# barrust/pyprobables

Measured on AMD Instinct MI355X. Metric: million keys/sec insert+lookup (Bloom m=2^28 k=7, CMS 2^20x5), higher is better.
Workload: dtype u64; 1 GPU; cfg2 Bloom m=2^28 k=7: per rank per step clear + insert 10M 16B keys + (merge) + check them; keys_per_rank=10000000, key_bytes=16, m_bits=268435456, k=7, parallelism=single GPU

## Files before the change

pyprobables_amd/csrc/psk_capi.hip:

```cpp
#include "psk_host.hpp"

#include <map>
#include <mutex>
#include <utility>

static thread_local char g_err[512] = "";

int fail(int code, const char *fmt, ...)
{
    va_list ap;
    va_start(ap, fmt);
    vsnprintf(g_err, sizeof(g_err), fmt, ap);
    va_end(ap);
    return code;
}


extern "C" const char *psk_last_error(void) { return g_err; }
extern "C" int psk_version(void) { return 100; }

extern "C" int psk_device_count(int *count)
{
    if (!count) return fail(PSK_EINVAL, "count is NULL");
    int n = 0;
// ... 317 lines not shown
    if (logical_bytes) *logical_bytes = s->logical_bytes;
    return PSK_OK;
}

extern "C" int psk_read_table(psk_sketch *s, void *dst_host, uint64_t nbytes, void *stream)
{
    CHECK_HANDLE_RO(s, -1);
    if (!dst_host || nbytes > s->padded_bytes) return fail(PSK_EINVAL, "bad read_table arguments");
    hipStream_t st = (hipStream_t)stream;
    PSK_TRY(flush_combined(s, st));
    HIP_TRY(hipMemcpyAsync(dst_host, s->table, nbytes, hipMemcpyDeviceToHost, st));
    HIP_TRY(hipStreamSynchronize(st));
    return PSK_OK;
}

extern "C" int psk_write_table(psk_sketch *s, const void *src_host, uint64_t nbytes, void *stream)
{
    CHECK_HANDLE(s, -1);
    if (!src_host || nbytes > s->padded_bytes) return fail(PSK_EINVAL, "bad write_table arguments");
    hipStream_t st = (hipStream_t)stream;
    PSK_TRY(drop_pending(s, st));
    s->clear_pending = false;
    HIP_TRY(hipMemsetAsync(s->table, 0, s->padded_bytes, st));
    HIP_TRY(hipMemcpyAsync(s->table, src_host, nbytes, hipMemcpyHostToDevice, st));
    HIP_TRY(hipMemsetAsync(s->ctr, 0, sizeof(long long) * PSK_CTR_COUNT, st));
    if (s->kind != PSK_KIND_BLOOM) {
        const uint64_t nel = s->logical_bytes / 4;
        hipLaunchKernelGGL(k_absmax, dim3(grid_for_keys(nel)), dim3(kBlock), 0, st, (const uint32_t *)s->table, nel,
                           s->kind == PSK_KIND_CMS ? 1 : 0, s->ctr);
        HIP_TRY(hipGetLastError());
    }
    HIP_TRY(hipStreamSynchronize(st));
    return PSK_OK;
}

extern "C" int psk_rescan_bound(psk_sketch *s, void *stream)
{
    CHECK_HANDLE(s, -1);
    if (s->owns_table || s->table_private) s->shadow.exposed = false;
    if (s->kind == PSK_KIND_BLOOM) return PSK_OK;
    hipStream_t st = (hipStream_t)stream;
    PSK_TRY(flush_combined(s, st));
    HIP_TRY(hipMemsetAsync(s->ctr + PSK_CTR_ABS_BOUND, 0, sizeof(long long), st));
    const uint64_t nel = s->logical_bytes / 4;
    hipLaunchKernelGGL(k_absmax, dim3(grid_for_keys(nel)), dim3(kBlock), 0, st, (const uint32_t *)s->table, nel,
                       s->kind == PSK_KIND_CMS ? 1 : 0, s->ctr);
    HIP_TRY(hipGetLastError());
    return PSK_OK;
}

extern "C" int psk_get_counters(psk_sketch *s, int64_t out[PSK_CTR_COUNT], void *stream)
{
    CHECK_HANDLE_RO(s, -1);
    if (!out) return fail(PSK_EINVAL, "out is NULL");
    hipStream_t st = (hipStream_t)stream;
    PSK_TRY(flush_combined(s, st));
    HIP_TRY(hipMemcpyAsync(out, s->ctr, sizeof(long long) * PSK_CTR_COUNT, hipMemcpyDeviceToHost, st));
    HIP_TRY(hipStreamSynchronize(st));
    return PSK_OK;
}

extern "C" int psk_reset_counters(psk_sketch *s, void *stream)
{
    CHECK_HANDLE(s, -1);
    HIP_TRY(hipMemsetAsync(s->ctr, 0, sizeof(long long) * PSK_CTR_ABS_BOUND, (hipStream_t)stream));
    return PSK_OK;
}

int raise_dyn_lds(const void *kernel, size_t bytes)
{
    static std::mutex mu;
    static std::map<std::pair<const void *, int>, size_t> granted;
    int dev = 0;
    HIP_TRY(hipGetDevice(&dev));
    std::lock_guard<std::mutex> lock(mu);
    size_t &have = granted[{kernel, dev}];
    if (bytes > have) {
        HIP_TRY(hipFuncSetAttribute(kernel, hipFuncAttributeMaxDynamicSharedMemorySize, (int)bytes));
        have = bytes;
    }
    return PSK_OK;
}

extern "C" int psk_set_option(const char *name, int64_t value)
{
    if (!name) return fail(PSK_EINVAL, "option name is NULL");
    const OptDesc *d = opt_find(name);
    if (!d || d->cls == kOptReadOnly) return fail(PSK_EINVAL, d ? "option %s is read-only" : "unknown option %s", name);
    if (value < d->lo) value = d->lo;
    __atomic_store_n(d->var, value, __ATOMIC_RELAXED);
    return PSK_OK;
}

extern "C" int psk_debug_phase_profile(psk_sketch *s, uint32_t nbuckets, uint32_t nwg, uint64_t out[12])
{
    if (!s || !s->s_cnt.p) return fail(PSK_EINVAL, "no partition scratch yet");
    PSK_USE_DEVICE(s->device);
    HIP_TRY(hipDeviceSynchronize());
    char *p = (char *)s->s_cnt.p + (size_t)nbuckets * nwg * 4;
    HIP_TRY(hipMemcpy(out, p, 96, hipMemcpyDeviceToHost));
    HIP_TRY(hipMemset(p, 0, 96));
    return PSK_OK;
}

extern "C" int psk_sketch_set_option(psk_sketch *s, const char *name, int64_t value)
{
    if (!s || !name) return fail(PSK_EINVAL, "NULL argument");
    if (!strcmp(name, "table_private")) {
        s->table_private = value != 0;
        if (s->table_private) s->shadow.exposed = false;
        else if (!s->owns_table) s->shadow.exposed = true;
        if (s->shadow.exposed && s->clear_pending) {
            PSK_USE_DEVICE(s->device);
            PSK_TRY(clear_materialize(s, nullptr));
        }
        ++s->table_version;
        return PSK_OK;
    }
    const OptDesc *d = opt_find(name);
    if (!d || d->ho < 0) return fail(PSK_EINVAL, "%s is not a per-sketch option", name);
    if (value != kHoUnset && value < d->lo) value = d->lo;
    s->opt[d->ho] = value;
    return PSK_OK;
}

extern "C" int psk_sketch_get_option(psk_sketch *s, const char *name, int64_t *value)
{
    if (!s || !name || !value) return fail(PSK_EINVAL, "NULL argument");
    if (!strcmp(name, "table_private")) {
        *value = s->table_private ? 1 : 0;
        return PSK_OK;
    }
    if (!strcmp(name, "window_pending_batches")) {
        *value = s->win.n ? (int64_t)s->win.batches.size() : 0;
        return PSK_OK;
    }
    const OptDesc *d = opt_find(name);
    if (!d || d->ho < 0) return fail(PSK_EINVAL, "%s is not a per-sketch option", name);
    *value = s->opt[d->ho] != kHoUnset ? s->opt[d->ho] : __atomic_load_n(d->var, __ATOMIC_RELAXED);
    return PSK_OK;
}

extern "C" int psk_get_option(const char *name, int64_t *value)
{
    if (!name || !value) return fail(PSK_EINVAL, "NULL argument");
    const OptDesc *d = opt_find(name);
    if (!d) return fail(PSK_EINVAL, "unknown option %s", name);
    *value = __atomic_load_n(d->var, __ATOMIC_RELAXED);
    return PSK_OK;
}

extern "C" int psk_scratch_bytes(psk_sketch *s, uint64_t bytes[3])
{
    if (!s || !bytes) return fail(PSK_EINVAL, "psk_scratch_bytes: NULL argument");
    uint64_t all = 0, waiting = 0;
    (void)for_each_scratch(s, [&](DevBuf &b, bool is_waiting) {
        if (b.p) all += b.cap;
        if (b.p && is_waiting) waiting += b.cap;
        return (int)PSK_OK;
    });
    bytes[0] = all;
    bytes[1] = waiting;
    bytes[2] = s->shadow.img.p ? s->shadow.img.cap : 0;
    return PSK_OK;
}

// ... 18 lines not shown
```

pyprobables_amd/csrc/psk_cbf.hip:

```cpp
#include "psk_stage.hpp"
#include "psk_nibble.hpp"
#include "psk_window.hpp"

static int cbf_apply_direct(psk_sketch *s, const Batch &b, const uint32_t *w, bool remove, hipStream_t st)
{
    unsigned long long *sat = (unsigned long long *)(s->ctr + PSK_CTR_SATURATED);
    return with_source(b, [&](auto src) {
        return with_pow2(s, [&](auto P) {
            if (remove) return launch_apply(src, CbfSub<P.value>{(uint32_t *)s->table, s->md, s->k, w, sat - 1}, b.n, st);
            return launch_apply(src, CbfAdd<P.value>{(uint32_t *)s->table, s->md, s->k, w, s->ctr, sat, false}, b.n, st);
        });
    });
}

static int cbf_apply_device(psk_sketch *s, const Batch &b, const uint32_t *w, bool remove, hipStream_t st)
{
    if (b.n == 0) return PSK_OK;
    PSK_TRY(post_acct(s, w, b.n, remove ? PSK_CTR_REMOVED : PSK_CTR_ADDED, (long long)s->k, st, !remove, false));
    bool done = false;
    PSK_TRY(remove ? cbf_remove_partitioned(s, b, w, st, &done, 0, nullptr) : cbf_add_partitioned(s, b, w, st, &done));
    PSK_TRY(settle_acct(s, w, b.n, st));
    if (done) return PSK_OK;
    return cbf_apply_direct(s, b, w, remove, st);
}

static int comb_order(psk_sketch *s, hipStream_t st)
{
    if (!s->scat.appended || st == s->scat.last) return PSK_OK;
    if (!s->scat.ev) HIP_TRY(hipEventCreateWithFlags(&s->scat.ev, hipEventDisableTiming));
    HIP_TRY(hipEventRecord(s->scat.ev, s->scat.last));
    HIP_TRY(hipStreamWaitEvent(st, s->scat.ev, 0));
    s->scat.last = st;
    return PSK_OK;
}

static int comb_appended(psk_sketch *s, hipStream_t st)
{
    s->scat.last = st;
    s->scat.appended = true;
    return PSK_OK;
}

static bool older_updates_pending(const psk_sketch *s)
{
    return s->comb.add.n || s->comb.rem.n || s->comb.badd.n() || s->comb.brem.n() || (s->scat.ready && s->scat.add.n);
}

static int scat_zero(psk_sketch *s, hipStream_t st)
{
    const uint64_t nseg = (uint64_t)s->scat.g.nbuckets * s->scat.g.nwg;
    if (!s->scat.add.cnt.p) return PSK_OK;
    hipLaunchKernelGGL(k_zero_u32, dim3(256), dim3(256), 0, st, (uint32_t *)s->scat.add.cnt.p, nseg);
    HIP_TRY(hipGetLastError());
    return PSK_OK;
}

static int scat_drop(psk_sketch *s, hipStream_t st)
{
    if (!s->scat.ready || s->scat.add.n == 0) return PSK_OK;
    PSK_TRY(comb_order(s, st));
    PSK_TRY(scat_zero(s, st));
    s->scat.add.n = 0;
    return PSK_OK;
}

int drop_pending(psk_sketch *s, hipStream_t st)
{
    s->comb.add.n = s->comb.rem.n = 0;
    s->comb.add.unit = s->comb.rem.unit = true;
    s->comb.badd.clear();
    s->comb.brem.clear();
    s->win.n = s->win.copied = 0;
    s->win.batches.clear();
    return scat_drop(s, st);
}

static int scat_flush(psk_sketch *s, hipStream_t st)
{
    if (!s->scat.ready || s->scat.add.n == 0) return PSK_OK;
    PSK_TRY(comb_order(s, st));
    const uint64_t na = s->scat.add.n;
    s->scat.add.n = 0;
    PartGeom g = s->scat.g;
    const uint64_t per_seg = (uint64_t)g.nbuckets * g.nwg * 6;
    g.dense = (na * s->k / per_seg) < (uint64_t)g_part_dense_groups ? 1u : 0u;
    const size_t lds = (size_t)1 << (g.shift - 1);
    unsigned long long *sat = (unsigned long long *)(s->ctr + PSK_CTR_SATURATED);
    const uint32_t direct = na * s->k >= s->m / 8 ? 0u : 1u;
    PSK_TRY(set_dyn_lds(k_nib_apply<0>, lds));
    hipLaunchKernelGGL(k_nib_apply<0>, dim3(g.nbuckets), dim3(kApplyThreads), lds, st, (uint32_t *)s->table, s->m, g, (const uint32_t *)s->scat.add.cnt.p,
                       (const uint4 *)s->scat.add.part.p, sat, direct);
    HIP_TRY(hipGetLastError());
    return scat_zero(s, st);
}

static int scat_append(psk_sketch *s, const Batch &b, uint64_t cap, hipStream_t st, bool *done)
{
    *done = false;
    {
        const uint64_t by_table = s->m * 5 / (2 * (uint64_t)(s->k ? s->k : 1));
        if (cap > by_table) cap = by_table;
    }
    if (s->kind != PSK_KIND_CBF || g_update_nibble == 0 || b.n == 0 || b.n > cap || s->k > 32) return PSK_OK;
    if (b.layout == PSK_KEYS_HASHES && b.key_len < s->k) return PSK_OK;
    if (!s->scat.ready || s->scat.cap != cap) {
        PartGeom g;
        if (!scat_geometry(s, cap, &g)) return PSK_OK;
        PSK_TRY(scat_flush(s, st));
        s->scat.g = g;
        s->scat.cap = cap;
        s->scat.ready = true;
    }
    psk_sketch::ScatList &l = s->scat.add;
    if (l.n + b.n > cap) PSK_TRY(flush_combined(s, st));
    const PartGeom &g = s->scat.g;
    const uint64_t part_bytes = (uint64_t)g.nbuckets * g.nwg * g.segcap * 16 + 256, cnt_bytes = (uint64_t)g.nbuckets * g.nwg * 4 + 128;
    if (l.part.cap < part_bytes || l.cnt.cap < cnt_bytes) {
        if (s->eff[HO_SCRATCH_BUDGET] > 0 && (int64_t)(part_bytes + cnt_bytes) > s->eff[HO_SCRATCH_BUDGET]) return PSK_OK;
        if (ensure(l.part, part_bytes) != PSK_OK || ensure(l.cnt, cnt_bytes) != PSK_OK) return PSK_OK;
        HIP_TRY(hipMemsetAsync(l.cnt.p, 0, cnt_bytes, st));
        l.n = 0;
    }
    PSK_TRY(comb_order(s, st));
    bool appended = false;
    PSK_TRY(cbf_scat_append(s, b, st, &appended));
    if (!appended) return PSK_OK;
    l.n += b.n;
    PSK_TRY(comb_appended(s, st));
    *done = true;
    return PSK_OK;
}

static int borrowed_flush(psk_sketch *s, psk_sketch::BorrowList &bl, bool remove, hipStream_t st)
{
    const uint64_t n = bl.n();
    if (n == 0) return PSK_OK;
    const uint32_t nb = (uint32_t)bl.base.size();
    PSK_TRY(ensure(s->s_brw, (uint64_t)(2 * nb + 2) * 8));
    const void **base_dev = (const void **)s->s_brw.p;
    uint64_t *start_dev = (uint64_t *)s->s_brw.p + nb;
    HIP_TRY(hipMemcpyAsync(base_dev, bl.base.data(), (size_t)nb * 8, hipMemcpyHostToDevice, st));
    HIP_TRY(hipMemcpyAsync(start_dev, bl.start.data(), (size_t)(nb + 1) * 8, hipMemcpyHostToDevice, st));
    HIP_TRY(hipStreamSynchronize(st));
    std::vector<const void *> bases;
    std::vector<uint64_t> starts;
    bases.swap(bl.base);
    starts.swap(bl.start);
    bl.clear();
    PSK_TRY(account_weights(s, (const uint32_t *)nullptr, n, remove ? PSK_CTR_REMOVED : PSK_CTR_ADDED, (long long)s->k, st, !remove));
    bool done = false;
    PSK_TRY(cbf_unit_multi_partitioned(s, (const void *const *)base_dev, start_dev, nb, n, remove ? 1 : 0, st, &done));
    if (done) return PSK_OK;
    for (uint32_t j = 0; j < nb; ++j) {
        const Batch b{PSK_KEYS_FIXED, bases[j], nullptr, starts[j + 1] - starts[j], 16};
        PSK_TRY(cbf_apply_direct(s, b, nullptr, remove, st));
    }
    return PSK_OK;
}

constexpr size_t kWinMaxBatches = 4096;

static uint64_t win_capacity(const psk_sketch *s)
{
    uint64_t cap = s->m / 2;
    if (cap < (1u << 20)) cap = 1u << 20;
    if (s->eff[HO_WINDOW_KEYS] > 0 && cap > (uint64_t)s->eff[HO_WINDOW_KEYS]) cap = (uint64_t)s->eff[HO_WINDOW_KEYS];
    cap = cap_round_by_budget(s, cap, 16.0 + (double)s->k * (16.0 / 6.0) * 1.5);
    return cap;
// ... 491 lines not shown
```

pyprobables_amd/csrc/psk_host.hpp:

```cpp
#pragma once
#include "psk_device.hpp"
#include "psk_partition.hpp"
#include "psk_part_bins.hpp"

#include <hip/hip_runtime.h>

#include <cstdarg>
#include <cstdio>
#include <cstdlib>
#include <cstring>
#include <new>
#include <type_traits>
#include <vector>

#include "../../include/psk.h"

using namespace psk;

#define PSK_HIDDEN __attribute__((visibility("hidden")))

PSK_HIDDEN int fail(int code, const char *fmt, ...);

#define HIP_TRY(expr)                                                                                   \
    do {                                                                                                \
// ... 158 lines not shown
        bool active = false, scattered = false;
        Batch b{};
        PartGeom g{};
        uint64_t round_keys = 0;
        int scheme = 0;
        uint32_t gen = 0;
    } pend;
};

PSK_HIDDEN int ensure(DevBuf &b, uint64_t bytes);

PSK_HIDDEN void resolve_options(psk_sketch *s);
#define CHECK_HANDLE_RO(s, want_kind)                                                    \
    do {                                                                                 \
        if (!(s)) return fail(PSK_EINVAL, "sketch handle is NULL");                      \
        if ((want_kind) >= 0 && (s)->kind != (want_kind))                                \
            return fail(PSK_EINVAL, "wrong sketch kind %d for this call", (s)->kind);    \
        resolve_options(s);                                                              \
    } while (0);                                                                         \
    PSK_USE_DEVICE((s)->device)
#define CHECK_HANDLE(s, want_kind)                                                       \
    CHECK_HANDLE_RO(s, want_kind);                                                       \
    ++(s)->table_version

static inline int grid_for_keys(uint64_t n)
{
    uint64_t g = (n + kBlock - 1) / kBlock;
    const uint64_t cap = 256ULL * 16;
    if (g > cap) g = cap;
    return (int)(g ? g : 1);
}


extern PSK_HIDDEN int64_t g_part_mode, g_part_max_keys, g_part_cache_bytes, g_part_two_level_slices, g_part_debug, g_part_tile_threads,
    g_part_even_tiles, g_part_dense_groups, g_part_bins, g_ragged_sort, g_lookup_half, g_lookup_nibble, g_update_nibble, g_nib_min_lg_lookup,
    g_nib_min_lg_update, g_small_weights, g_remove_dryrun, g_combine_keys, g_auto_combine_keys, g_window_wide, g_window_tile,
    g_window_force_fail, g_merge_single_rank, g_lazy_clear, g_host_poll_us,
    g_cbf_ordered_replays, g_window_folds, g_window_replays, g_small_weights_used, g_cbf_shadow_hits, g_running_fast, g_running_sequential,
    g_update_running_fast, g_update_running_sequential;

static inline bool part_slices(uint64_t cells, uint32_t max_shift, uint32_t min_shift, PartGeom *g,
                               uint64_t max_buckets = kPartMaxBuckets, int target_lg = 8)
{
    if (cells >= (1ULL << 32) || cells < (1ULL << 16)) return false;
    const uint32_t lg = 63 - __builtin_clzll(cells);
    int shift = (int)lg - target_lg;
    if (shift > (int)max_shift) shift = max_shift;
    if (shift < (int)min_shift) shift = min_shift;
    const uint64_t B = (cells + (1ULL << shift) - 1) >> shift;
    if (B > max_buckets) return false;
    g->nbuckets = (uint32_t)B;
    g->shift = (uint32_t)shift;
    g->dbg = (uint32_t)g_part_debug | (g_ragged_sort == 0 ? kGeomNoSortBit : 0u);
    g->split = g->split_idx = 0;
    g->dense = 0;
    g->append = 0;
    return true;
}

static inline bool nib_geometry(uint64_t cells, bool update, PartGeom *g)
{
    if (update ? cells <= (1ULL << g_nib_min_lg_update) : cells < (1ULL << g_nib_min_lg_lookup)) return false;
    return part_slices(cells, kNibShift, 15, g, kPartMaxBuckets, 8);
}

static inline bool nib_load_ok(uint64_t n, uint32_t k, uint64_t cells) { return n * (uint64_t)k * 2 <= cells * 5; }

static inline bool scat_geometry(const psk_sketch *s, uint64_t cap, PartGeom *g)
{
    if (!nib_geometry(s->m, true, g)) return false;
    g->k = s->k;
    g->nwg = 256;
    g->append = 1;
    g->tile = 0;
    const double tile_keys = 2048.0 * 7.0 / (double)(s->k < 1 ? 1 : s->k);
    const double mean = (double)cap * s->k / ((double)g->nbuckets * g->nwg);
    const double runs = 2.0 * (double)cap / (tile_keys * g->nwg) + 64.0;
    const double segcap = mean / 6.0 + 0.5 * runs + 8.0 * __builtin_sqrt(mean) / 6.0 + 16.0;
    if (segcap >= (double)(1u << 24) || (double)g->nbuckets * segcap >= 4294967296.0) return false;
    g->segcap = (uint32_t)segcap;
    return true;
}

PSK_HIDDEN int raise_dyn_lds(const void *kernel, size_t bytes);

template <class K>
static int set_dyn_lds(K kernel, size_t bytes)
{
    return raise_dyn_lds((const void *)kernel, bytes);
}

template <class Pay, int KT, int NT>
static size_t scatter_lds_bytes(const PartGeom *g, uint64_t tile = 0, bool sorted = false)
{
    if (sorted) return scatter_lds_bytes<Pay, KT, NT>(g, tile, false) + 16 + 8 * (size_t)kSortBins + 18 * (size_t)PartTile<Pay, KT, NT>::TILE;
    using Tile = PartTile<Pay, KT, NT>;
    const uint32_t kk = g->k < (uint32_t)KT ? g->k : (uint32_t)KT;
    const size_t tk = tile ? (size_t)tile : (size_t)Tile::TILE;
    const size_t stage_cap = ((tk * kk + (size_t)(Tile::GS - 1) * g->nbuckets) + 3) & ~(size_t)3;
    const size_t stage_words = stage_cap + (Tile::pair ? stage_cap / Tile::GS + 4 : 0);
    return (5 * (size_t)g->nbuckets + 16 + 24 + stage_words) * 4;
}

struct ScatterTarget {
    uint32_t *cnt;
    uint4 *part;
};

#ifndef PSK_LOOKUP_FAT_SLICES
#define PSK_LOOKUP_FAT_SLICES 900
#endif
constexpr uint32_t kLookupFatSlices = PSK_LOOKUP_FAT_SLICES;
constexpr size_t kScatterLdsBudget = 160 * 1024;
constexpr size_t kScatterLdsTwoPerCu = 78 * 1024;

template <class Src>
struct src_fat512 { static constexpr bool value = std::is_same<Src, KeysFixed16>::value || std::is_same<Src, KeysFixed16Multi>::value || std::is_same<Src, KeysFixed8>::value; };

template <class Src, class Pay, int KT>
struct bins_eligible {
    static constexpr bool value = pay_bins_ok<Pay>::value && KT <= 8 && src_fat512<Src>::value;
};
#ifndef PSK_BINS_CARRY_GROUP
#define PSK_BINS_CARRY_GROUP 1
#endif
constexpr size_t kBinSlackWords = 8 + 16;
struct BinsPlan {
    uint32_t tile, cap, stride, per_cu;
    size_t lds;
};
template <int KT>
static bool bins_plan(const PartGeom *g, BinsPlan *p)
{
    if (g_part_bins == 0 || g->nbuckets > (uint32_t)kBinThreads * kBinSlicesPerLane || g->nbuckets < 2) return false;
    constexpr double kSigmas = 3.5;
    const uint32_t kk = g->k < (uint32_t)KT ? g->k : (uint32_t)KT;
    p->tile = (uint32_t)kBinThreads * kBinKpt;
    const double mean = (double)p->tile * kk / (double)g->nbuckets;
    uint32_t cap = (uint32_t)(mean + kSigmas * __builtin_sqrt(mean) + 2.0);
    cap = (cap + 5) / 6 * 6;
    auto plan = [&](uint32_t c) {
        uint32_t stride = kBinHead + c + 1;
        while (stride % 4 != 2) ++stride;
        const size_t lds = ((size_t)g->nbuckets * stride + kBinSlackWords) * 4;
        if (lds > kScatterLdsBudget / 2) return false;
        p->cap = c;
        p->stride = stride;
        p->lds = lds;
        return true;
    };
    if (!(PSK_BINS_CARRY_GROUP && plan(cap + 6)) && !plan(cap)) return false;
    uint32_t per_cu = (uint32_t)(kScatterLdsBudget / p->lds);
    const uint32_t by_waves = 2048u / (uint32_t)kBinThreads;
    p->per_cu = per_cu > by_waves ? by_waves : per_cu;
    return true;
}

template <class Src, class IdxFn, class Pay, class Spill, int KT>
static int launch_scatter_bins(psk_sketch *s, const Src &src, const IdxFn &idxfn, const Pay &pay, const Spill &spill, PartGeom *g, uint64_t n,
                               hipStream_t st, uint32_t want_wgs, const BinsPlan &bp)
{
    const uint32_t kk = g->k < (uint32_t)KT ? g->k : (uint32_t)KT;
    const uint64_t tile_full = bp.tile;
    const uint64_t ntiles = (n + tile_full - 1) / tile_full;
    uint64_t nwg = 256ULL * bp.per_cu;
    if (want_wgs) nwg = want_wgs;
    if (nwg > 64u * kApplyWaves) nwg = 64u * kApplyWaves;
    if (nwg > ntiles) nwg = ntiles;
    if (nwg == 0) nwg = 1;
    const uint64_t tiles_per_wg = (ntiles + nwg - 1) / nwg;
    uint64_t tk = tile_full;
    if (g_part_even_tiles != 0 && nwg * tiles_per_wg > ntiles) {
        tk = ((n + nwg * tiles_per_wg - 1) / (nwg * tiles_per_wg) + 63) & ~63ULL;
        if (tk > tile_full) tk = tile_full;
    }
    const double mean = (double)tiles_per_wg * (double)tk * kk / (double)g->nbuckets;
    uint64_t segcap = (uint64_t)(mean / 6.0 + 0.5 * (double)tiles_per_wg + 8.0 * __builtin_sqrt(mean) / 6.0 + 16.0);
    if constexpr (pay_tile_tag<Pay>::value) {
        if (tiles_per_wg > 16) return fail(PSK_EINVAL, "lookup round of %llu keys needs %llu tiles per workgroup (max 16)",
                                           (unsigned long long)n, (unsigned long long)tiles_per_wg);
    }
    if (segcap >= (1u << 24) || (uint64_t)g->nbuckets * segcap >= (1ULL << 32))
        return fail(PSK_EINVAL, "partition round of %llu keys is too large (segments of %llu groups)", (unsigned long long)n, (unsigned long long)segcap);
    g->nwg = (uint32_t)nwg;
    g->segcap = (uint32_t)segcap;
    g->tile = (uint32_t)tk;
    g->dense = (mean / 6.0 + 0.5 * (double)tiles_per_wg) < (double)g_part_dense_groups ? 1u : 0u;
    PSK_TRY(ensure(s->s_part, (uint64_t)g->nbuckets * nwg * segcap * 16 + 256));
    PSK_TRY(ensure(s->s_cnt, (uint64_t)g->nbuckets * nwg * 4 + 128));
    auto kern = k_part_bins<Src, IdxFn, Pay, Spill, KT, kBinKpt>;
    PSK_TRY(set_dyn_lds(kern, bp.lds));
    hipLaunchKernelGGL(kern, dim3((unsigned)nwg), dim3(kBinThreads), bp.lds, st, src, idxfn, pay, spill, *g, (uint32_t)n, bp.cap, bp.stride,
                       (uint32_t *)s->s_cnt.p, (uint4 *)s->s_part.p);
    HIP_TRY(hipGetLastError());
    return PSK_OK;
}
template <class Src, class IdxFn, class Pay, class Spill, int KT, int NT>
static int launch_scatter_nt(psk_sketch *s, const Src &src, const IdxFn &idxfn, const Pay &pay, const Spill &spill, PartGeom *g,
                             uint64_t n, hipStream_t st, uint32_t want_wgs, const ScatterTarget *fixed = nullptr)
{
    if constexpr (bins_eligible<Src, Pay, KT>::value) {
        BinsPlan bp;
        if (!fixed && n < (1ULL << 31) && bins_plan<KT>(g, &bp)) return launch_scatter_bins<Src, IdxFn, Pay, Spill, KT>(s, src, idxfn, pay, spill, g, n, st, want_wgs, bp);
    }
    using Tile = PartTile<Pay, KT, NT>;
    constexpr bool kSorted = src_sorted<Src>::value;
    const uint32_t kk = g->k < (uint32_t)KT ? g->k : (uint32_t)KT;
    uint64_t tile_full = Tile::TILE;
    if constexpr (pay_is_lookup<Pay>::value && pay_fat1024<Pay>::value) {
        if (g->nbuckets < kLookupFatSlices && tile_full > 2048) tile_full = 2048;
    }
    while (tile_full > 64 && scatter_lds_bytes<Pay, KT, NT>(g, tile_full, kSorted) > kScatterLdsBudget) tile_full -= 64;
    if (scatter_lds_bytes<Pay, KT, NT>(g, tile_full, kSorted) > kScatterLdsBudget) return fail(PSK_EINVAL, "pass 1: %u slices do not fit the LDS stage", g->nbuckets);
    const uint64_t ntiles = (n + tile_full - 1) / tile_full;
    if (fixed) {
        if (Pay::mode != kModePlain) return fail(PSK_EINVAL, "persistent segments carry payload-free probes");
        const uint64_t grid = g->nwg < ntiles ? g->nwg : ntiles;
        if (grid == 0) return PSK_OK;
        const uint64_t per_wg = (ntiles + grid - 1) / grid;
        uint64_t tk = tile_full;
        if (g_part_even_tiles != 0 && grid * per_wg > ntiles) {
            tk = ((n + grid * per_wg - 1) / (grid * per_wg) + 63) & ~63ULL;
            if (tk > tile_full) tk = tile_full;
        }
        g->tile = (uint32_t)tk;
        const size_t lds = scatter_lds_bytes<Pay, KT, NT>(g, tk, kSorted);
        auto kern = k_part_scatter<Src, IdxFn, Pay, Spill, KT, NT>;
        PSK_TRY(set_dyn_lds(kern, lds));
        hipLaunchKernelGGL(kern, dim3((unsigned)grid), dim3(NT), lds, st, src, idxfn, pay, spill, *g, n, fixed->cnt, fixed->part);
        HIP_TRY(hipGetLastError());
        return PSK_OK;
    }
    uint64_t per_cu = NT > 512 ? 1 : (scatter_lds_bytes<Pay, KT, NT>(g, tile_full, kSorted) > kScatterLdsTwoPerCu ? 1 : 2);
    if (kBenchKnobs && (g->dbg & 8)) per_cu = 1;
    uint64_t nwg = 256 * per_cu;
    if (want_wgs) nwg = want_wgs;
    if (nwg > 64u * kApplyWaves) nwg = 64u * kApplyWaves;
    if (nwg > ntiles) nwg = ntiles;
    const uint64_t tiles_per_wg = (ntiles + nwg - 1) / nwg;
    uint64_t tk = tile_full;
    if (g_part_even_tiles != 0 && nwg * tiles_per_wg > ntiles) {
        tk = ((n + nwg * tiles_per_wg - 1) / (nwg * tiles_per_wg) + 63) & ~63ULL;
        if (tk > tile_full) tk = tile_full;
    }
    const size_t lds = scatter_lds_bytes<Pay, KT, NT>(g, tk, kSorted);
    const double mean = (double)tiles_per_wg * (double)tk * kk / (double)g->nbuckets;
    uint64_t segcap = (uint64_t)(mean / Tile::GS + 0.5 * (double)tiles_per_wg + 8.0 * __builtin_sqrt(mean) / Tile::GS + 16.0);
    if constexpr (Pay::mode == kModeKeyed || pay_tile_tag<Pay>::value) {
        if (tiles_per_wg > 16) return fail(PSK_EINVAL, "lookup round of %llu keys needs %llu tiles per workgroup (max 16)",
                                           (unsigned long long)n, (unsigned long long)tiles_per_wg);
    }
    if (segcap >= (1u << 24) || (uint64_t)g->nbuckets * segcap >= (1ULL << 32))
        return fail(PSK_EINVAL, "partition round of %llu keys is too large (segments of %llu groups)", (unsigned long long)n, (unsigned long long)segcap);
    g->nwg = (uint32_t)nwg;
    g->segcap = (uint32_t)segcap;
    g->tile = (uint32_t)tk;
    g->dense = (mean / Tile::GS + 0.5 * (double)tiles_per_wg) < (double)g_part_dense_groups ? 1u : 0u;
    PSK_TRY(ensure(s->s_part, (uint64_t)g->nbuckets * nwg * segcap * 16 + 256));
    PSK_TRY(ensure(s->s_cnt, (uint64_t)g->nbuckets * nwg * 4 + 128));
    auto kern = k_part_scatter<Src, IdxFn, Pay, Spill, KT, NT>;
    PSK_TRY(set_dyn_lds(kern, lds));
    hipLaunchKernelGGL(kern, dim3((unsigned)nwg), dim3(NT), lds, st, src, idxfn, pay, spill, *g, n, (uint32_t *)s->s_cnt.p,
                       (uint4 *)s->s_part.p);
    HIP_TRY(hipGetLastError());
    return PSK_OK;
}


template <class Pay, int KT, bool FAT = true>
static int scatter_threads(const PartGeom *g)
{
    if constexpr (!FAT && (pay_fat512<Pay>::value || pay_fat1024<Pay>::value)) return scatter_threads<PaySlim<Pay>, KT, false>(g);
    if constexpr (KT <= 8 && !(pay_fat512<Pay>::value && FAT)) return 1024;
    if constexpr (KT <= 8) {
        const bool fits1024 = scatter_lds_bytes<Pay, KT, 1024>(g, PartTile<Pay, KT, 1024>::TILE > 2048 ? 2048 : 0) <= kScatterLdsBudget;
        const bool two_per_cu = pay_fat512<Pay>::value && scatter_lds_bytes<Pay, KT, kPartThreads>(g) <= kScatterLdsTwoPerCu;
        bool use1024 = fits1024 && !two_per_cu;
        if (g_part_tile_threads == 1024) use1024 = fits1024;
        if (g_part_tile_threads == 512 || (kBenchKnobs && (g->dbg & 16))) use1024 = false;
        if (use1024) return 1024;
    }
    return kPartThreads;
}
template <class Pay, int KT, bool FAT = true, bool SORTED = false>
static uint64_t scatter_round_cap(const PartGeom *g, uint32_t want_wgs, uint32_t max_tiles)
{
    if constexpr (!FAT && (pay_fat512<Pay>::value || pay_fat1024<Pay>::value)) return scatter_round_cap<PaySlim<Pay>, KT, false, SORTED>(g, want_wgs, max_tiles);
    if constexpr (pay_bins_ok<Pay>::value && KT <= 8 && FAT) {
        BinsPlan bp;
        if (bins_plan<KT>(g, &bp)) {
            uint64_t nwg = 256ULL * bp.per_cu;
            if (want_wgs) nwg = want_wgs;
            if (nwg > 64u * kApplyWaves) nwg = 64u * kApplyWaves;
            return nwg * max_tiles * bp.tile;
        }
    }
    const bool big = scatter_threads<Pay, KT, FAT>(g) == 1024;
    const size_t lds = big ? scatter_lds_bytes<Pay, KT, 1024>(g) : scatter_lds_bytes<Pay, KT, kPartThreads>(g);
    uint64_t tile = big ? (uint64_t)PartTile<Pay, KT, 1024>::TILE : (uint64_t)PartTile<Pay, KT, kPartThreads>::TILE;
    if (big) while (tile > 64 && scatter_lds_bytes<Pay, KT, 1024>(g, tile, SORTED) > kScatterLdsBudget) tile -= 64;
    else while (tile > 64 && scatter_lds_bytes<Pay, KT, kPartThreads>(g, tile, SORTED) > kScatterLdsBudget) tile -= 64;
    uint64_t nwg = 256 * (uint64_t)(big ? 1 : (lds > kScatterLdsTwoPerCu ? 1 : 2));
    if (kBenchKnobs && (g->dbg & 8)) nwg = 256;
    if (want_wgs) nwg = want_wgs;
    if (nwg > 64u * kApplyWaves) nwg = 64u * kApplyWaves;
    return nwg * max_tiles * tile;
}

template <class Src, class IdxFn, class Pay, class Spill, int KT>
static int launch_scatter(psk_sketch *s, const Src &src, const IdxFn &idxfn, const Pay &pay, const Spill &spill, PartGeom *g,
                          uint64_t n, hipStream_t st, uint32_t want_wgs = 0, const ScatterTarget *fixed = nullptr)
{
    if constexpr (!src_fat512<Src>::value && (pay_fat512<Pay>::value || pay_fat1024<Pay>::value))
        return launch_scatter<Src, IdxFn, PaySlim<Pay>, Spill, KT>(s, src, idxfn, PaySlim<Pay>(pay), spill, g, n, st, want_wgs, fixed);
    if constexpr (Pay::mode == kModeKeyed)
        static_assert(((uint64_t)PartTile<Pay, KT, kPartThreads>::TILE << Pay::slice_shift) <= (1ULL << 31),
                      "512-thread tiles must keep keyed probes inside 31 bits for the largest slice");
    if constexpr (KT <= 8) {
        if constexpr (Pay::mode == kModeKeyed)
            static_assert(((uint64_t)PartTile<Pay, KT, 1024>::TILE << Pay::slice_shift) <= (1ULL << 31), "keyed tile too large");
        if constexpr (!(pay_fat512<Pay>::value && src_fat512<Src>::value)) {
            return launch_scatter_nt<Src, IdxFn, Pay, Spill, KT, 1024>(s, src, idxfn, pay, spill, g, n, st, want_wgs, fixed);
        } else {
            if (scatter_threads<Pay, KT, true>(g) == 1024) return launch_scatter_nt<Src, IdxFn, Pay, Spill, KT, 1024>(s, src, idxfn, pay, spill, g, n, st, want_wgs, fixed);
            return launch_scatter_nt<Src, IdxFn, Pay, Spill, KT, kPartThreads>(s, src, idxfn, pay, spill, g, n, st, want_wgs, fixed);
        }
    } else {
        return launch_scatter_nt<Src, IdxFn, Pay, Spill, KT, kPartThreads>(s, src, idxfn, pay, spill, g, n, st, want_wgs, fixed);
    }
}

template <class Src, class F>
static int with_kt(uint32_t k, F &&f)
{
    constexpr bool fast16 = std::is_same<Src, KeysFixed16>::value || std::is_same<Src, KeysFixed16Multi>::value;
    constexpr bool fast2 = std::is_same<Src, KeysFixed8>::value || std::is_same<Src, KeysFixed32>::value || std::is_same<Src, KeysVarlen<uint8_t>>::value;
    if constexpr (fast16) {
        switch (k) {
            case 3: return f(std::integral_constant<int, 3>{});
            case 4: return f(std::integral_constant<int, 4>{});
// ... 165 lines not shown
```

pyprobables_amd/csrc/psk_partition.hpp:

```cpp
#pragma once
#include <type_traits>
#include "psk_device.hpp"

#ifndef PSK_BENCH_KNOBS
#define PSK_BENCH_KNOBS 0
#endif

namespace psk {

constexpr bool kBenchKnobs = PSK_BENCH_KNOBS != 0;
constexpr int kPartThreads = 512;
constexpr int kPartProbes = 32;
constexpr int kPartMaxBuckets = 2048;
constexpr int kPartScanPerThread = 4;
constexpr bool kPartPipeline = true;
constexpr bool kPartHash32 = true;
constexpr uint32_t kNibShift = 18;
constexpr uint32_t kGeomNoSortBit = 0x40000000u;
constexpr int kSortSub = 16;
constexpr int kSortBins = 64 * kSortSub;
constexpr uint32_t kPadProbe = 0xFFFFFFFFu;
#ifndef PSK_EXP_PRIO
#define PSK_EXP_PRIO 1
#endif
// ... 956 lines not shown
                if (pre[mid] <= f) lo = mid;
                else hi = mid;
            }
            q = buckets1[seg_index(g1, c, seg_lo + lo) * g1.segcap + (f - pre[lo])];
        }
        const uint32_t e[4] = {q.x, q.y, q.z, q.w};
        uint32_t rank[4];
#pragma unroll
        for (int j = 0; j < 4; ++j)
            if (e[j] != kPadProbe) rank[j] = atomicAdd(&hist[(e[j] & mask1) >> g2.shift], 1u);
        __syncthreads();
        if (threadIdx.x < 64) {
            const uint32_t cnt = threadIdx.x < S ? hist[threadIdx.x] : 0;
            const uint32_t padded = (cnt + GS - 1) / GS * GS;
            const uint32_t inc = wave_inclusive_scan(padded);
            if (threadIdx.x < S) {
                const uint32_t at = inc - padded;
                off[threadIdx.x] = at;
                const uint32_t c0 = cur[threadIdx.x];
                delta[threadIdx.x] = c0 - at / GS;
                cur[threadIdx.x] = c0 + padded / GS;
                for (uint32_t x = cnt; x < padded; ++x) stage[at + x] = kPadProbe;
            }
            if (threadIdx.x == 63) total_probes = inc;
        }
        __syncthreads();
#pragma unroll
        for (int j = 0; j < 4; ++j)
            if (e[j] != kPadProbe) stage[off[(e[j] & mask1) >> g2.shift] + rank[j]] = e[j];
        __syncthreads();
        const uint32_t out_groups = total_probes / GS;
        for (uint32_t gi = threadIdx.x; gi < out_groups; gi += NT) {
            uint32_t v[GS];
#pragma unroll
            for (int x = 0; x < GS; ++x) v[x] = stage[gi * GS + x];
            const uint32_t sub = (v[0] & mask1) >> g2.shift;
            const uint32_t slice = (c << sub_bits) + sub;
            const uint32_t slot = delta[sub] + gi;
            if (slot < g2.segcap) {
                uint4 o;
                if constexpr (OUT == 0) {
                    uint32_t nv = 0;
#pragma unroll
                    for (int x = 0; x < 6; ++x) nv += v[x] != kPadProbe;
                    const uint32_t n0 = nv < 3 ? nv : 3, n1 = nv - n0;
                    auto l = [&](int x) -> unsigned long long { return (uint32_t)x < nv ? (unsigned long long)(v[x] & mask) : 0ULL; };
                    const unsigned long long h0 = l(0) | (l(1) << 20) | (l(2) << 40) | ((unsigned long long)n0 << 60);
                    const unsigned long long h1 = l(3) | (l(4) << 20) | (l(5) << 40) | ((unsigned long long)n1 << 60);
                    o = make_uint4((uint32_t)h0, (uint32_t)(h0 >> 32), (uint32_t)h1, (uint32_t)(h1 >> 32));
                } else if constexpr (OUT == 1) {
                    auto h16 = [&](int x) -> uint32_t { return v[x] == kPadProbe ? 0xFFFFu : (v[x] & mask); };
                    o = make_uint4(h16(0) | (h16(1) << 16), h16(2) | (h16(3) << 16), h16(4) | (h16(5) << 16), h16(6) | (h16(7) << 16));
                } else {
                    auto w32 = [&](int x) -> uint32_t { return v[x] == kPadProbe ? kPadProbe : (((v[x] >> g1.shift) << g2.shift) | (v[x] & mask)); };
                    o = make_uint4(w32(0), w32(1), w32(2), w32(3));
                }
                buckets2[seg_index(g2, slice, p) * g2.segcap + slot] = o;
            } else {
#pragma unroll
                for (int x = 0; x < GS; ++x)
                    if (v[x] != kPadProbe) spill((slice << g2.shift) | (v[x] & mask), v[x] >> g1.shift);
            }
        }
        __syncthreads();
    }
    if (threadIdx.x < S) {
        const uint32_t slice = (c << sub_bits) + threadIdx.x;
        if (slice < g2.nbuckets) segcnt2[(uint64_t)slice * g2.nwg + p] = cur[threadIdx.x] < g2.segcap ? cur[threadIdx.x] : g2.segcap;
    }
}

constexpr int kApplyThreads = 1024;
constexpr int kApplyWaves = kApplyThreads / 64;

__device__ __forceinline__ uint32_t lane_segment_count(const uint32_t *segcnt, const PartGeom &g, uint32_t b)
{
    const uint32_t lane = threadIdx.x & 63, wave = threadIdx.x >> 6;
    const uint32_t S = g.split > 1 ? g.split : 1, s0 = g.split > 1 ? g.split_idx : 0;
    const uint32_t mine_total = g.nwg > s0 ? (g.nwg - s0 + S - 1) / S : 0;
    const uint32_t nseg = mine_total > wave ? (mine_total - wave + kApplyWaves - 1) / kApplyWaves : 0;
    return lane < nseg ? segcnt[(uint64_t)b * g.nwg + s0 + S * (wave + kApplyWaves * lane)] : 0u;
}

template <int D, class Body>
__device__ __forceinline__ void for_each_batch_at(const uint4 *buckets, const uint32_t *segcnt, const PartGeom &g, uint32_t b,
                                                  const uint4 pad, Body body, uint32_t mycnt_pre = ~0u)
{
    const uint32_t lane = threadIdx.x & 63, wave = threadIdx.x >> 6;
    const uint32_t S = g.split > 1 ? g.split : 1, s0 = g.split > 1 ? g.split_idx : 0;
    const uint32_t mycnt = mycnt_pre != ~0u ? mycnt_pre : lane_segment_count(segcnt, g, b);
    if (g.dense) {
        const uint32_t incl = wave_inclusive_scan(mycnt), excl = incl - mycnt;
        const uint32_t T = (uint32_t)__builtin_amdgcn_readlane((int)incl, 63);
        for (uint32_t G0 = 0; G0 < T; G0 += 64u * D) {
            uint4 q[D];
            uint64_t at[D];
            uint32_t wg[D];
#pragma unroll
            for (int d = 0; d < D; ++d) {
                const uint32_t row = G0 + 64u * (uint32_t)d;
                const uint32_t G = row + lane;
                uint32_t t = (uint32_t)__builtin_popcountll(__ballot(incl <= row));
                const uint32_t sl = t < 64 ? t : 63;
                uint32_t seg = sl;
                uint32_t first = (uint32_t)__builtin_amdgcn_readlane((int)excl, sl);
                for (; t < 64; ++t) {
                    const uint32_t end_t = (uint32_t)__builtin_amdgcn_readlane((int)incl, t);
                    if (end_t > row + 63u) break;
                    const bool past = G >= end_t;
                    seg = past ? t + 1 : seg;
                    first = past ? end_t : first;
                }
                seg = seg < 64 ? seg : 63;
                wg[d] = s0 + S * (wave + kApplyWaves * seg);
                q[d] = pad;
                at[d] = ~0ULL;
                if (G < T) {
                    const uint64_t idx = seg_index(g, b, wg[d]) * g.segcap + (G - first);
                    q[d] = buckets[idx];
                    at[d] = idx;
                }
            }
            body(q, at, wg);
        }
        return;
    }
    const uint32_t chunks = (mycnt + 63) >> 6;
    const uint32_t incl = wave_inclusive_scan(chunks), excl = incl - chunks;
    const uint32_t C = (uint32_t)__builtin_amdgcn_readlane((int)incl, 63);
    for (uint32_t c0 = 0; c0 < C; c0 += D) {
        uint4 q[D];
        uint64_t at[D];
        uint32_t wg[D];
#pragma unroll
        for (int d = 0; d < D; ++d) {
            const uint32_t cc = c0 + d;
            const uint32_t seg = (uint32_t)__builtin_popcountll(__ballot(incl <= cc));
            const uint32_t sl = seg < 64 ? seg : 63;
            const uint32_t v = (cc - (uint32_t)__builtin_amdgcn_readlane((int)excl, sl)) * 64 + lane;
            const uint32_t cnt = seg < 64 ? (uint32_t)__builtin_amdgcn_readlane((int)mycnt, sl) : 0;
            wg[d] = s0 + S * (wave + kApplyWaves * sl);
            const uint64_t base = seg_index(g, b, wg[d]) * g.segcap;
            q[d] = pad;
            at[d] = ~0ULL;
            if (v < cnt) {
                q[d] = buckets[base + v];
                at[d] = base + v;
            }
        }
        body(q, at, wg);
    }
}

template <int D, class Body>
__device__ __forceinline__ void for_each_batch(const uint4 *buckets, const uint32_t *segcnt, const PartGeom &g, uint32_t b,
                                               const uint4 pad, Body body)
{
    const uint32_t lane = threadIdx.x & 63, wave = threadIdx.x >> 6;
    const uint32_t nseg = g.nwg > wave ? (g.nwg - wave + kApplyWaves - 1) / kApplyWaves : 0;
    uint32_t mycnt = 0;
    if (lane < nseg) mycnt = segcnt[(uint64_t)b * g.nwg + wave + kApplyWaves * lane];
    if (g.dense) {
        const uint32_t incl = wave_inclusive_scan(mycnt), excl = incl - mycnt;
        const uint32_t T = (uint32_t)__builtin_amdgcn_readlane((int)incl, 63);
        for (uint32_t G0 = 0; G0 < T; G0 += 64u * D) {
            uint4 q[D];
#pragma unroll
            for (int d = 0; d < D; ++d) {
                const uint32_t row = G0 + 64u * (uint32_t)d;
                const uint32_t G = row + lane;
                uint32_t t = (uint32_t)__builtin_popcountll(__ballot(incl <= row));
                const uint32_t sl = t < 64 ? t : 63;
                uint32_t seg = sl;
                uint32_t first = (uint32_t)__builtin_amdgcn_readlane((int)excl, sl);
                for (; t < 64; ++t) {
                    const uint32_t end_t = (uint32_t)__builtin_amdgcn_readlane((int)incl, t);
                    if (end_t > row + 63u) break;
                    const bool past = G >= end_t;
                    seg = past ? t + 1 : seg;
                    first = past ? end_t : first;
                }
                seg = seg < 64 ? seg : 63;
                q[d] = pad;
                if (G < T) q[d] = buckets[seg_index(g, b, wave + kApplyWaves * seg) * g.segcap + (G - first)];
            }
            body(q);
        }
        return;
    }
    const uint32_t chunks = (mycnt + 63) >> 6;
    const uint32_t incl = wave_inclusive_scan(chunks), excl = incl - chunks;
    const uint32_t C = (uint32_t)__builtin_amdgcn_readlane((int)incl, 63);
    for (uint32_t c0 = 0; c0 < C; c0 += D) {
        uint4 q[D];
#pragma unroll
        for (int d = 0; d < D; ++d) {
            const uint32_t cc = c0 + d;
            const uint32_t seg = (uint32_t)__builtin_popcountll(__ballot(incl <= cc));
            const uint32_t sl = seg < 64 ? seg : 63;
            const uint32_t v = (cc - (uint32_t)__builtin_amdgcn_readlane((int)excl, sl)) * 64 + lane;
            const uint32_t cnt = seg < 64 ? (uint32_t)__builtin_amdgcn_readlane((int)mycnt, sl) : 0;
            const uint4 *src = buckets + seg_index(g, b, wave + kApplyWaves * sl) * g.segcap;
            q[d] = pad;
            if (v < cnt) q[d] = src[v];
        }
        body(q);
    }
}

constexpr int kApplyDepth = 12;

constexpr uint64_t kNtTableWords = 1ULL << 25;
__device__ __forceinline__ uint4 slice_piece(const uint32_t *tab, uint64_t tab_words, uint64_t w0, uint32_t w, bool nt = false)
{
    const uint64_t gw = w0 + w;
    if (gw + 3 < tab_words) {
        if (nt) {
            typedef unsigned int nt_u32x4 __attribute__((ext_vector_type(4)));
            const nt_u32x4 v = __builtin_nontemporal_load(reinterpret_cast<const nt_u32x4 *>(tab + gw));
            return make_uint4(v.x, v.y, v.z, v.w);
        }
        return *reinterpret_cast<const uint4 *>(tab + gw);
    }
    uint4 t = make_uint4(0, 0, 0, 0);
    if (gw + 0 < tab_words) t.x = tab[gw + 0];
    if (gw + 1 < tab_words) t.y = tab[gw + 1];
    if (gw + 2 < tab_words) t.z = tab[gw + 2];
    return t;
}

constexpr int kSliceLoads = 8;
__device__ __forceinline__ void load_slice(uint32_t *smem, const uint32_t *tab, uint64_t tab_words, uint64_t w0, uint32_t slice_words)
{
    const bool nt = tab_words >= kNtTableWords;
    for (uint32_t wb = threadIdx.x * 4; wb < slice_words; wb += kApplyThreads * 4 * kSliceLoads) {
        uint4 t[kSliceLoads];
#pragma unroll
        for (int u = 0; u < kSliceLoads; ++u) {
            const uint32_t w = wb + (uint32_t)u * kApplyThreads * 4;
            t[u] = w < slice_words ? slice_piece(tab, tab_words, w0, w, nt) : make_uint4(0, 0, 0, 0);
        }
#pragma unroll
        for (int u = 0; u < kSliceLoads; ++u) {
            const uint32_t w = wb + (uint32_t)u * kApplyThreads * 4;
            if (w < slice_words) *reinterpret_cast<uint4 *>(smem + w) = t[u];
        }
    }
}

template <int DEPTH = kApplyDepth, class F4>
__device__ __forceinline__ void for_each_group(const uint4 *buckets, const uint32_t *segcnt, const PartGeom &g, uint32_t b,
                                               const uint4 pad, F4 f4)
{
    for_each_batch<DEPTH>(buckets, segcnt, g, b, pad, [&](const uint4 (&q)[DEPTH]) {
#pragma unroll
        for (int d = 0; d < DEPTH; ++d) f4(q[d]);
    });
}

template <class Pre, class Post>
__device__ __forceinline__ void for_each_group_padded(const uint4 *buckets, const uint32_t *segcnt, const PartGeom &g, uint32_t b,
                                                      const uint4 pad, Pre pre, Post post)
{
    for_each_batch<kApplyDepth>(buckets, segcnt, g, b, pad, [&](const uint4 (&q)[kApplyDepth]) {
        uint4 w[kApplyDepth];
#pragma unroll
        for (int d = 0; d < kApplyDepth; ++d) w[d] = pre(q[d]);
// ... 464 lines not shown
```

Before: 60900 Mkeys/s.

## Add fast two-segment dense row walk and cost-based dense walk selection

Adds a dense_row helper for the pass-2 bucket walk. When a 64-lane row covers at most two segments, it computes addresses with wave-uniform scalar values and skips the per-lane segment search loop. It also replaces the fixed threshold that enables dense mode with a heuristic that compares chunked versus dense row counts per wave, so dense mode can also turn on at higher loads. The risk is that dense mode now runs in regimes where its per-row setup costs more than chunked iteration would, and the base_b address arithmetic depends on assumptions about segment stride layout.

```diff
diff --git a/pyprobables_amd/csrc/psk_capi.hip b/pyprobables_amd/csrc/psk_capi.hip
--- a/pyprobables_amd/csrc/psk_capi.hip
+++ b/pyprobables_amd/csrc/psk_capi.hip
@@ -423,6 +423,17 @@
     return PSK_OK;
 }
 
+constexpr double kDenseWalkRowMargin = 1.25;
+uint32_t pass2_walk_dense(double mean_groups, uint32_t nwg)
+{
+    if (g_part_dense_groups <= 0) return 0u;
+    if (mean_groups < (double)g_part_dense_groups) return 1u;
+    double per_wave = (double)((nwg + kApplyWaves - 1) / kApplyWaves);
+    if (per_wave < 1.0) per_wave = 1.0;
+    const double chunked = per_wave * __builtin_ceil(mean_groups / 64.0), dense = __builtin_ceil(per_wave * mean_groups / 64.0);
+    return chunked >= kDenseWalkRowMargin * dense ? 1u : 0u;
+}
+
 extern "C" int psk_set_option(const char *name, int64_t value)
 {
     if (!name) return fail(PSK_EINVAL, "option name is NULL");
diff --git a/pyprobables_amd/csrc/psk_cbf.hip b/pyprobables_amd/csrc/psk_cbf.hip
--- a/pyprobables_amd/csrc/psk_cbf.hip
+++ b/pyprobables_amd/csrc/psk_cbf.hip
@@ -83,7 +83,7 @@
     s->scat.add.n = 0;
     PartGeom g = s->scat.g;
     const uint64_t per_seg = (uint64_t)g.nbuckets * g.nwg * 6;
-    g.dense = (na * s->k / per_seg) < (uint64_t)g_part_dense_groups ? 1u : 0u;
+    g.dense = pass2_walk_dense((double)(na * s->k / per_seg), g.nwg);
     const size_t lds = (size_t)1 << (g.shift - 1);
     unsigned long long *sat = (unsigned long long *)(s->ctr + PSK_CTR_SATURATED);
     const uint32_t direct = na * s->k >= s->m / 8 ? 0u : 1u;
diff --git a/pyprobables_amd/csrc/psk_host.hpp b/pyprobables_amd/csrc/psk_host.hpp
--- a/pyprobables_amd/csrc/psk_host.hpp
+++ b/pyprobables_amd/csrc/psk_host.hpp
@@ -264,6 +264,8 @@
     return true;
 }
 
+PSK_HIDDEN uint32_t pass2_walk_dense(double mean_groups, uint32_t nwg);
+
 PSK_HIDDEN int raise_dyn_lds(const void *kernel, size_t bytes);
 
 template <class K>
@@ -367,7 +369,7 @@
     g->nwg = (uint32_t)nwg;
     g->segcap = (uint32_t)segcap;
     g->tile = (uint32_t)tk;
-    g->dense = (mean / 6.0 + 0.5 * (double)tiles_per_wg) < (double)g_part_dense_groups ? 1u : 0u;
+    g->dense = pass2_walk_dense(mean / 6.0 + 0.5 * (double)tiles_per_wg, (uint32_t)nwg);
     PSK_TRY(ensure(s->s_part, (uint64_t)g->nbuckets * nwg * segcap * 16 + 256));
     PSK_TRY(ensure(s->s_cnt, (uint64_t)g->nbuckets * nwg * 4 + 128));
     auto kern = k_part_bins<Src, IdxFn, Pay, Spill, KT, kBinKpt>;
@@ -437,7 +439,7 @@
     g->nwg = (uint32_t)nwg;
     g->segcap = (uint32_t)segcap;
     g->tile = (uint32_t)tk;
-    g->dense = (mean / Tile::GS + 0.5 * (double)tiles_per_wg) < (double)g_part_dense_groups ? 1u : 0u;
+    g->dense = pass2_walk_dense(mean / Tile::GS + 0.5 * (double)tiles_per_wg, (uint32_t)nwg);
     PSK_TRY(ensure(s->s_part, (uint64_t)g->nbuckets * nwg * segcap * 16 + 256));
     PSK_TRY(ensure(s->s_cnt, (uint64_t)g->nbuckets * nwg * 4 + 128));
     auto kern = k_part_scatter<Src, IdxFn, Pay, Spill, KT, NT>;
diff --git a/pyprobables_amd/csrc/psk_partition.hpp b/pyprobables_amd/csrc/psk_partition.hpp
--- a/pyprobables_amd/csrc/psk_partition.hpp
+++ b/pyprobables_amd/csrc/psk_partition.hpp
@@ -1062,6 +1062,29 @@
     return lane < nseg ? segcnt[(uint64_t)b * g.nwg + s0 + S * (wave + kApplyWaves * lane)] : 0u;
 }
 
+template <class Pair, class Mixed>
+__device__ __forceinline__ void dense_row(uint32_t incl, uint32_t excl, uint32_t T, uint32_t row, uint32_t lane, Pair pair, Mixed mixed)
+{
+    uint32_t t = (uint32_t)__builtin_popcountll(__ballot(incl <= row));
+    const uint32_t sl = t < 64 ? t : 63;
+    const uint32_t first_s = (uint32_t)__builtin_amdgcn_readlane((int)excl, sl);
+    const uint32_t end_next = sl < 63 ? (uint32_t)__builtin_amdgcn_readlane((int)incl, sl + 1) : T;
+    if (end_next > row + 63u || end_next == T) {
+        pair(sl, row - first_s, (uint32_t)__builtin_amdgcn_readlane((int)incl, sl) - row);
+        return;
+    }
+    const uint32_t G = row + lane;
+    uint32_t seg = sl, first = first_s;
+    for (; t < 64; ++t) {
+        const uint32_t end_t = (uint32_t)__builtin_amdgcn_readlane((int)incl, t);
+        if (end_t > row + 63u) break;
+        const bool past = G >= end_t;
+        seg = past ? t + 1 : seg;
+        first = past ? end_t : first;
+    }
+    mixed(seg < 64 ? seg : 63, G - first);
+}
+
 template <int D, class Body>
 __device__ __forceinline__ void for_each_batch_at(const uint4 *buckets, const uint32_t *segcnt, const PartGeom &g, uint32_t b,
                                                   const uint4 pad, Body body, uint32_t mycnt_pre = ~0u)
@@ -1070,6 +1093,8 @@
     const uint32_t S = g.split > 1 ? g.split : 1, s0 = g.split > 1 ? g.split_idx : 0;
     const uint32_t mycnt = mycnt_pre != ~0u ? mycnt_pre : lane_segment_count(segcnt, g, b);
     if (g.dense) {
+        const uint32_t wave_s = (uint32_t)__builtin_amdgcn_readfirstlane((int)wave);
+        const uint64_t seg_stride = (uint64_t)S * kApplyWaves * g.nbuckets * g.segcap;
         const uint32_t incl = wave_inclusive_scan(mycnt), excl = incl - mycnt;
         const uint32_t T = (uint32_t)__builtin_amdgcn_readlane((int)incl, 63);
         for (uint32_t G0 = 0; G0 < T; G0 += 64u * D) {
@@ -1079,27 +1104,28 @@
 #pragma unroll
             for (int d = 0; d < D; ++d) {
                 const uint32_t row = G0 + 64u * (uint32_t)d;
-                const uint32_t G = row + lane;
-                uint32_t t = (uint32_t)__builtin_popcountll(__ballot(incl <= row));
-                const uint32_t sl = t < 64 ? t : 63;
-                uint32_t seg = sl;
-                uint32_t first = (uint32_t)__builtin_amdgcn_readlane((int)excl, sl);
-                for (; t < 64; ++t) {
-                    const uint32_t end_t = (uint32_t)__builtin_amdgcn_readlane((int)incl, t);
-                    if (end_t > row + 63u) break;
-                    const bool past = G >= end_t;
-                    seg = past ? t + 1 : seg;
-                    first = past ? end_t : first;
-                }
-                seg = seg < 64 ? seg : 63;
-                wg[d] = s0 + S * (wave + kApplyWaves * seg);
                 q[d] = pad;
                 at[d] = ~0ULL;
-                if (G < T) {
-                    const uint64_t idx = seg_index(g, b, wg[d]) * g.segcap + (G - first);
-                    q[d] = buckets[idx];
-                    at[d] = idx;
-                }
+                dense_row(incl, excl, T, row, lane,
+                          [&](uint32_t seg, uint32_t off, uint32_t in_a) {
+                              const uint32_t wg_a = s0 + S * (wave_s + kApplyWaves * seg);
+                              const uint64_t seg_a = seg_index(g, b, wg_a) * g.segcap;
+                              const uint64_t base_a = seg_a + off, base_b = seg_a + seg_stride - in_a;
+                              const bool second = lane >= in_a;
+                              wg[d] = second ? wg_a + S * kApplyWaves : wg_a;
+                              if (row + lane < T) {
+                                  at[d] = (second ? base_b : base_a) + lane;
+                                  q[d] = buckets[at[d]];
+                              }
+                          },
+                          [&](uint32_t seg, uint32_t off) {
+                              wg[d] = s0 + S * (wave_s + kApplyWaves * seg);
+                              if (row + lane < T) {
+                                  const uint64_t idx = seg_index(g, b, wg[d]) * g.segcap + off;
+                                  q[d] = buckets[idx];
+                                  at[d] = idx;
+                              }
+                          });
             }
             body(q, at, wg);
         }
@@ -1141,6 +1167,8 @@
     uint32_t mycnt = 0;
     if (lane < nseg) mycnt = segcnt[(uint64_t)b * g.nwg + wave + kApplyWaves * lane];
     if (g.dense) {
+        const uint32_t wave_s = (uint32_t)__builtin_amdgcn_readfirstlane((int)wave);
+        const uint64_t seg_stride = (uint64_t)kApplyWaves * g.nbuckets * g.segcap;
         const uint32_t incl = wave_inclusive_scan(mycnt), excl = incl - mycnt;
         const uint32_t T = (uint32_t)__builtin_amdgcn_readlane((int)incl, 63);
         for (uint32_t G0 = 0; G0 < T; G0 += 64u * D) {
@@ -1148,21 +1176,16 @@
 #pragma unroll
             for (int d = 0; d < D; ++d) {
                 const uint32_t row = G0 + 64u * (uint32_t)d;
-                const uint32_t G = row + lane;
-                uint32_t t = (uint32_t)__builtin_popcountll(__ballot(incl <= row));
-                const uint32_t sl = t < 64 ? t : 63;
-                uint32_t seg = sl;
-                uint32_t first = (uint32_t)__builtin_amdgcn_readlane((int)excl, sl);
-                for (; t < 64; ++t) {
-                    const uint32_t end_t = (uint32_t)__builtin_amdgcn_readlane((int)incl, t);
-                    if (end_t > row + 63u) break;
-                    const bool past = G >= end_t;
-                    seg = past ? t + 1 : seg;
-                    first = past ? end_t : first;
-                }
-                seg = seg < 64 ? seg : 63;
                 q[d] = pad;
-                if (G < T) q[d] = buckets[seg_index(g, b, wave + kApplyWaves * seg) * g.segcap + (G - first)];
+                dense_row(incl, excl, T, row, lane,
+                          [&](uint32_t seg, uint32_t off, uint32_t in_a) {
+                              const uint64_t seg_a = seg_index(g, b, wave_s + kApplyWaves * seg) * g.segcap;
+                              const uint64_t base_a = seg_a + off, base_b = seg_a + seg_stride - in_a;
+                              if (row + lane < T) q[d] = buckets[(lane >= in_a ? base_b : base_a) + lane];
+                          },
+                          [&](uint32_t seg, uint32_t off) {
+                              if (row + lane < T) q[d] = buckets[seg_index(g, b, wave_s + kApplyWaves * seg) * g.segcap + off];
+                          });
             }
             body(q);
         }
```

Result: no change. 62300 Mkeys/s, median of 5 (+2.3%).
